# watsonyanghx/GAN_Lib_Tensorflow

Hardware: AMD Instinct MI355X
Metric: images/sec (G+D step) SNGAN-ResNet CIFAR-10 bs=64 (higher is better)
Workload: dtype bf16; 1 GPU; SNGAN ResNet CIFAR-10 32x32 bs=64 hinge: 1 G update (2x64 fakes) + 5 D updates (64 real + 64 fake) per step; global_batch=64, per_gpu_batch=64, parallelism=dp1, graphs=True, finite=True, collectives_in_graphs=False, grad_wire=fp32

## Files before the change

### gan_lib_tensorflow_amd/_lib.py

```python
import ctypes as C
import os

_HERE = os.path.dirname(os.path.abspath(__file__))
DTYPE = os.environ.get("GANK_DTYPE", "bf16").lower()
if DTYPE not in ("bf16", "fp16"):
    raise RuntimeError(f"GANK_DTYPE={DTYPE!r}: bf16 or fp16")
ACT_DTYPE_NAME = "bfloat16" if DTYPE == "bf16" else "float16"
LIB_PATH = os.path.join(_HERE, os.environ.get("GANK_LIB_NAME", "libgank.so" if DTYPE == "bf16" else "libgank_f16.so"))

P, I, L, F = C.c_void_p, C.c_int, C.c_long, C.c_float

IN_UPSAMPLE2X, IN_RELU, OUT_TANH, DY_UPSAMPLE2X, RES_UPSAMPLE2X, STATS_PREZEROED, OUT_POOLSUM2X = 1, 2, 4, 8, 64, 256, 512
STAT_SLOTS = 16


class SnDesc(C.Structure):
    _fields_ = [(n, P) for n in ("W", "u_in", "u_out", "v", "W_bar", "scal", "a", "b", "bpart",
                                 "dW_bar", "dW", "rowdot", "ga", "u_snap")] + \
               [("K", I), ("C", I), ("row_offset", I), ("chunk_offset", I)]


class WgradItem(C.Structure):
    _fields_ = [("x", P), ("dy", P), ("dw", P), ("dbias", P)]

# ... 64 lines not shown
    "gank_res8_chain_bwd_head": [C.POINTER(Res8Head), P, P, P, P, P, P, P, I, I, I, P],
    "gank_res8_conv3x3": [P, P, P, P, P, I, I, I, I, P, I, P],
    "gank_im2col_narrow": [P, P, I, I, I, I, I, I, I, I, I, I, P],
    "gank_tap_gather_up2": [P, P, P, I, I, I, I, I, I, I, I, P],
    "gank_tap_scatter_up2": [P, P, I, I, I, I, I, I, I, P],
    "gank_depth_to_space2": [P, P, I, I, I, I, P],
    "gank_space_to_depth2": [P, P, I, I, I, I, P],
    "gank_cpool_res_fprop": [P, P, P, P, P, I, I, I, I, I, I, P],
    "gank_cpool_res_dgrad": [P, P, P, P, I, I, I, I, I, P],
    "gank_cpool_res_dgrad_image_wgrad": [P, P, P, P, P, P, P, P, P, I, I, I, I, I, P, P],
    "gank_sum_slabs": [C.POINTER(SlabJob), I, P],
    "gank_convpool3x3_wgrad_job": [P, P, P, P, P, L, I, I, I, I, I, I, C.POINTER(SlabJob), P],
    "gank_conv2d_wgrad_slab_elems": [I, I, I, I, I, I, I],
    "gank_conv2d_wgrad_slabs": [P, P, P, P, I, I, I, I, I, I, I, F, P, L, C.POINTER(SlabJob), P],
    "gank_conv2d_wgrad_slab_splits": [I, I, I, I, I, I, I],
    "gank_conv2d_wgrad_slabs_rows": [P, P, P, P, I, I, I, I, I, I, I, I, F, P, L, C.POINTER(SlabJob), P],
    "gank_conv2d_wgrad_slabs_rows_tap_sums": [P, P, P, P, I, I, I, I, I, I, I, I, F, P, L, C.POINTER(SlabJob), P, I, P, P],
    "gank_conv2d_wgrad_batched_ws_elems": [I, I, I, I, I, I, I, I],
    "gank_conv2d_wgrad_batched_slabs": [C.POINTER(WgradItem), I, I, I, I, I, I, I, I, F, P, L, C.POINTER(SlabJob), P],
    "gank_deconv2d_prep_phases": [P, P, I, I, I, P],
    "gank_deconv2d_fprop": [P, P, P, P, I, I, I, I, I, I, P],
    "gank_deconv2d_dgrad": [P, P, P, I, I, I, I, I, I, P],
    "gank_deconv2d_wgrad": [P, P, P, I, I, I, I, I, I, P],
    "gank_colsum_bf16": [P, P, L, I, F, P],
    "gank_sn_ws_floats": [I, I],
    "gank_sn_power_iter_fwd": [C.POINTER(SnDesc), I, P],
    "gank_sn_power_iter_bwd": [C.POINTER(SnDesc), I, P],
    "gank_sn_power_iter_fwd_prep": [C.POINTER(SnDesc), I, C.POINTER(PrepDesc), C.POINTER(C.c_int), I, C.POINTER(LabelDenseDesc), P],
    "gank_sn_power_iter_fwd_a": [C.POINTER(SnDesc), I, P],
    "gank_sn_power_iter_fwd_b_prep": [C.POINTER(SnDesc), I, C.POINTER(PrepDesc), C.POINTER(C.c_int), I, C.POINTER(LabelDenseDesc), P, P, P, I, P],
    "gank_sn_power_iter_fwd_b_prep_feed": [C.POINTER(SnDesc), I, C.POINTER(PrepDesc), C.POINTER(C.c_int), I, C.POINTER(LabelDenseDesc), P, P, P, I,
                                           C.POINTER(CriticFeedDesc), P],
    "gank_sn_power_iter_bwd_gw": [C.POINTER(SnDesc), I, P],
    "gank_sn_adam_fwd_a": [C.POINTER(SnDesc), I, C.POINTER(C.c_void_p), P, P, P, P, L, P, P, P, P, I, P, P, P],
    "gank_label_dense_table": [P, P, P, P, P, I, I, I, P],
    "gank_concat_label_fwd": [P, P, P, P, I, I, I, I, I, P],
    "gank_concat_label_bwd": [P, P, P, I, I, I, I, P],
    "gank_label_dense_bwd": [P, P, P, P, P, P, P, I, I, I, I, P],
    "gank_label_conv3x3_bwd_pooled": [P, P, P, I, P, I, I, I, I, I, P, P, P, P, I, I, I, P],
    "gank_label_dense_bwd_parts": [P, I, P, P, P, P, P, I, I, I, P],
    "gank_sum_slabs_label_bwd": [P, I, P, P, P, I, P, I, I, I, I, I, P, P, P, I, I, I, P],
    "gank_concat_label_pool_fwd": [P, P, P, P, P, I, I, I, I, I, I, P],
    "gank_concat_label_unpool_bwd": [P, P, P, P, I, I, I, I, I, P],
    "gank_concat_label_unpool_bwd_factored": [P, P, P, P, P, I, P, P, I, I, I, I, I, I, P],
    "gank_label_conv3x3_table": [P, I, I, I, I, P, I, P, P, P, I, P, P],
    "gank_label_conv3x3_table_pooled": [P, I, I, I, I, P, I, P, P, P, I, P, P, P, I, I, I, P],
    "gank_label_conv3x3_table_pooled_shortcut": [P, I, I, I, I, P, I, P, P, P, I, P, P, P, I, I, I, P, I, P, I, P, P],
    "gank_img16_conv3x3_label_bias": [P, P, P, P, I, P, I, I, I, I, P],
    "gank_img16_conv3x3_dgrad_unpool": [P, P, P, P, I, F, P, I, I, I, P],
    "gank_img16_conv3x3_label_bwd": [P, P, P, P, I, I, I, I, P, P, I, P, I, I, I, I, P, P, P],
    "gank_label_conv3x3_bwd_ws_floats": [I, I],
    "gank_label_conv3x3_bwd": [P, P, P, I, P, I, I, I, I, I, I, I, P, P, P, P, P],
    "gank_cbn_parts": [L],
    "gank_cbn_fwd": [P, P, P, P, P, P, P, I, I, I, I, I, I, P],
    "gank_cbn_fwd_from_sums": [P, P, P, P, P, P, P, P, I, I, I, I, I, I, F, P],
    "gank_cbn_fwd_eps": [P, P, P, P, P, P, P, I, I, I, I, I, I, F, P],
    "gank_layer_norm_fwd": [P, P, P, P, P, I, I, I, F, P],
    "gank_layer_norm_bwd": [P, P, P, P, P, P, P, I, I, I, P],
    "gank_pixel_norm_fwd": [P, P, L, I, F, P],
    "gank_pixel_norm_bwd": [P, P, P, L, I, F, P],
    "gank_cbn_bwd": [P, P, P, P, P, P, P, P, P, P, I, I, I, I, I, I, P],
    "gank_cbn_stats": [P, P, P, I, I, I, I, F, P],
    "gank_cbn_stats_from_sums": [P, P, P, I, I, L, F, P],
    "gank_cbn_relu_conv3x3_fprop": [P, P, P, P, P, P, P, P, I, I, I, I, I, I, I, I, P],
    "gank_cbn_bwd_remask": [P, P, P, P, P, P, P, P, P, P, I, I, I, I, I, I, P],
    "gank_cbn_bwd_ws_floats": [I, I, I, I],
# ... 107 lines not shown
```

### gan_lib_tensorflow_amd/csrc/elementwise.hip

```cpp
#include "gank_common.h"
#include "label_conv_dev.h"

static inline dim3 grid1d(long n, int block = 256, int cap = 4096) {
  long g = (n + block - 1) / block;
  if (g > cap) g = cap;
  if (g < 1) g = 1;
  return dim3((unsigned)g);
}

#include "prep_weights.h"

__global__ void prep_wf_kernel(const float* __restrict__ w, bf16* __restrict__ wf, int K, int Cout, int CoutPad, int Kpad) {
  __shared__ float t[32][33];
  const int k0 = blockIdx.x * 32, c0 = blockIdx.y * 32;
  const int tx = threadIdx.x & 31, ty = threadIdx.x >> 5;
  for (int i = ty; i < 32; i += 8) {
    const int k = k0 + i, c = c0 + tx;
    t[i][tx] = (k < K && c < Cout) ? w[(long)k * Cout + c] : 0.f;
  }
  __syncthreads();
  for (int i = ty; i < 32; i += 8) {
    const int c = c0 + i, k = k0 + tx;
    if (c < CoutPad && k < Kpad) wf[(long)c * Kpad + k] = f2bf(t[tx][i]);
  }
}

__global__ void prep_wd_kernel(const float* __restrict__ w, bf16* __restrict__ wd, int taps, int Cin, int Cout, int CinPad, int Kpad2) {
  const long total = (long)CinPad * Kpad2;
  for (long i = blockIdx.x * (long)blockDim.x + threadIdx.x; i < total; i += (long)gridDim.x * blockDim.x) {
    const int ci = (int)(i / Kpad2), k = (int)(i - (long)ci * Kpad2);
    float v = 0.f;
    if (ci < Cin && k < taps * Cout) {
      const int tp = k / Cout, co = k - tp * Cout;
      v = w[((long)(taps - 1 - tp) * Cin + ci) * Cout + co];
// ... 820 lines not shown
    if (g < cg1) {
      bf16x8 o;
#pragma unroll
      for (int e = 0; e < 8; e++) o[e] = f2bf(v[e]);
      *reinterpret_cast<bf16x8*>(da + ((long)n * HW + r) * C1 + g * 8) = o;
    } else {
#pragma unroll
      for (int e = 0; e < 8; e++) acc[e] += bf2f(f2bf(v[e]));
    }
  }
#pragma unroll
  for (int e = 0; e < 8; e++) red[threadIdx.x * 8 + e] = acc[e];
  __syncthreads();
  for (int c = threadIdx.x; c < C2; c += NT) {
    const int gg = cg1 + (c >> 3);
    float t = 0.f;
    for (int l = 0; l < RL; l++) t += red[(l * cg + gg) * 8 + (c & 7)];
    if (de_parts > 0) {
      int lb = labels[n];
      lb = lb < 0 ? 0 : (lb >= V ? V - 1 : lb);
      if (lists[(long)lb * (N + 1) + 1] == n)
        for (int p = 0; p < de_parts; p++) t += de_add[((long)p * V + lb) * C2 + c];
    }
    de[(long)n * C2 + c] = t;
  }
  (void)cg2;
}

__global__ __launch_bounds__(1024) void label_dense_bwd_kernel(const float* __restrict__ de, const int* __restrict__ labels,
                                                               const float* __restrict__ table, const float* __restrict__ W,
                                                               float* __restrict__ dW, float* __restrict__ dbias, float* __restrict__ dtable,
                                                               int N, int V, int D, int C2, const float* __restrict__ de_add, int de_parts) {
  extern __shared__ __attribute__((aligned(16))) float lds_f[];
  float* dTg = lds_f;
  float* dT = dTg + 1024 * V;
  int* lbs = reinterpret_cast<int*>(dT + ((V * C2 + 3) & ~3));
  float* Ws = reinterpret_cast<float*>(lbs + ((N + 3) & ~3));
  float* Es = Ws + 8 * C2;
  float* dto = Es + 8 * V;
  const int tid = threadIdx.x, lane = tid & 63, wave = tid >> 6;
  const int NG = 1024 / C2, j = tid % C2, g = tid / C2;
  const int k0 = blockIdx.x * 8;
  float dw_old = 0.f, dt_old = 0.f, db_old = 0.f;
  if (dW && tid < 8 * C2 && k0 + tid / C2 < D) dw_old = dW[(long)(k0 + tid / C2) * C2 + tid % C2];
  if (dtable && tid < 8 * V && k0 + (tid & 7) < D) dt_old = dtable[(long)(tid >> 3) * D + k0 + (tid & 7)];
  if (dbias && blockIdx.x == 0 && tid < C2) db_old = dbias[tid];
  if (N == 0) {
    for (int idx = tid; idx < V * C2; idx += 1024) {
      float t = 0.f;
      for (int p = 0; p < de_parts; p++) t += de_add[(long)p * V * C2 + idx];
      dT[idx] = t;
    }
  }
  if (N > 0)
    for (int l = 0; l < V; l++) dTg[(g * V + l) * C2 + j] = 0.f;
  for (int i = tid; i < N; i += 1024) lbs[i] = labels[i];
  if (W)
    for (int i = tid; i < 8 * C2; i += 1024) { const int k = k0 + i / C2; Ws[i] = k < D ? W[(long)k * C2 + i % C2] : 0.f; }
  if (table)
    for (int i = tid; i < 8 * V; i += 1024) { const int k = k0 + (i & 7), l = i >> 3; Es[i] = k < D ? bf2f(f2bf(table[(long)l * D + k])) : 0.f; }
  __syncthreads();
  for (int nb = g; nb < N; nb += 16 * NG) {
    float x[16];
#pragma unroll
    for (int u = 0; u < 16; u++) {
      const int n = nb + u * NG;
      x[u] = n < N ? de[(long)n * C2 + j] : 0.f;
    }
#pragma unroll
    for (int u = 0; u < 16; u++) {
      const int n = nb + u * NG;
      const int l = n < N ? lbs[n] : -1;
      if (l >= 0 && l < V) dTg[(g * V + l) * C2 + j] += x[u];
    }
  }
  __syncthreads();
  if (N > 0) {
    for (int idx = tid; idx < V * C2; idx += 1024) {
      const int l = idx / C2, jj = idx % C2;
      float t = 0.f;
      for (int gg = 0; gg < NG; gg++) t += dTg[(gg * V + l) * C2 + jj];
      for (int p = 0; p < de_parts; p++) t += de_add[((long)p * V + l) * C2 + jj];
      dT[idx] = t;
    }
    __syncthreads();
  }
  if (dW)
    for (int i = tid; i < 8 * C2; i += 1024) {
      const int kk = i / C2, jj = i % C2;
      if (k0 + kk < D) {
        float t = 0.f;
        for (int l = 0; l < V; l++) t += Es[l * 8 + kk] * dT[l * C2 + jj];
        dW[(long)(k0 + kk) * C2 + jj] = (i == tid ? dw_old : dW[(long)(k0 + kk) * C2 + jj]) + t;
      }
    }
  if (dtable) {
    for (int p = wave; p < 8 * V; p += 16) {
      const int kk = p & 7, l = p >> 3;
      float t = 0.f;
      for (int jj = lane; jj < C2; jj += 64) t += dT[l * C2 + jj] * Ws[kk * C2 + jj];
      t = wave_sum(t);
      if (lane == 0) dto[p] = t;
    }
    __syncthreads();
    for (int p = tid; p < 8 * V; p += 1024) {
      const int kk = p & 7, l = p >> 3;
      if (k0 + kk < D) dtable[(long)l * D + k0 + kk] = (p == tid ? dt_old : dtable[(long)l * D + k0 + kk]) + dto[p];
    }
  }
  if (dbias && blockIdx.x == 0)
    for (int jj = tid; jj < C2; jj += 1024) {
      float t = 0.f;
      for (int l = 0; l < V; l++) t += dT[l * C2 + jj];
      dbias[jj] = (jj == tid ? db_old : dbias[jj]) + t;
    }
}

extern "C" int gank_concat_label_fwd(const void* a, const void* T, const int32_t* labels, void* y, int N, int HW, int C1, int C2, int V,
                                     void* stream) {
  GANK_REQUIRE(a && T && labels && y && N > 0 && HW > 0 && V > 0, "concat_label_fwd: bad arguments");
  GANK_REQUIRE(C1 % 8 == 0 && C2 % 8 == 0, "concat_label_fwd: channel counts must be multiples of 8");
  const long total8 = (long)N * HW * ((C1 + C2) / 8);
  hipLaunchKernelGGL(concat_label_fwd_kernel, grid1d(total8), dim3(256), 0, (hipStream_t)stream, (const bf16*)a, (const bf16*)T, labels, (bf16*)y,
                     total8, HW, C1, C2, V);
  GANK_LAUNCH_OK("concat_label_fwd");
  return 0;
}
extern "C" int gank_concat_label_bwd(const void* dy, void* da, float* de32, int N, int HW, int C1, int C2, void* stream) {
  GANK_REQUIRE(dy && da && de32 && N > 0 && HW > 0, "concat_label_bwd: bad arguments");
  GANK_REQUIRE(C1 % 8 == 0 && C2 % 8 == 0 && 1024 % (C2 / 8) == 0, "concat_label_bwd: unsupported channel counts %d,%d", C1, C2);
  hipLaunchKernelGGL(concat_label_bwd_kernel, dim3(N), dim3(1024), 0, (hipStream_t)stream, (const bf16*)dy, (bf16*)da, de32, HW, C1, C2);
  GANK_LAUNCH_OK("concat_label_bwd");
  return 0;
}
extern "C" int gank_concat_label_pool_fwd(const void* a, const void* T, const int32_t* labels, void* y, void* y_pooled, int N, int H, int W,
                                          int C1, int C2, int V, void* stream) {
  GANK_REQUIRE(a && T && labels && y_pooled && N > 0 && H > 0 && W > 0 && V > 0, "concat_label_pool_fwd: bad arguments");
  GANK_REQUIRE(C1 % 8 == 0 && C2 % 8 == 0 && H % 2 == 0 && W % 2 == 0, "concat_label_pool_fwd: channel counts must be multiples of 8, the size even");
  const long total8 = (long)N * (H / 2) * (W / 2) * ((C1 + C2) / 8);
  hipLaunchKernelGGL(concat_label_pool_fwd_kernel, grid1d(total8), dim3(256), 0, (hipStream_t)stream, (const bf16*)a, (const bf16*)T, labels,
                     (bf16*)y, (bf16*)y_pooled, total8, H / 2, W / 2, C1, C2, V);
  GANK_LAUNCH_OK("concat_label_pool_fwd");
  return 0;
}
extern "C" int gank_concat_label_unpool_bwd(const void* g_main, const void* g_pooled, void* da, float* de32, int N, int H, int W, int C1, int C2,
                                            void* stream) {
  GANK_REQUIRE(g_pooled && da && de32 && N > 0 && H > 0 && W > 0, "concat_label_unpool_bwd: bad arguments");
  GANK_REQUIRE(C1 % 8 == 0 && C2 % 8 == 0 && H % 2 == 0 && W % 2 == 0 && 1024 % ((C1 + C2) / 8) == 0,
// ... 71 lines not shown
```

### gan_lib_tensorflow_amd/csrc/sn.hip

```cpp
#include "gank_common.h"
#include "prep_weights.h"
#include "feed.h"

#define SN_MAX 16
#define SN_EPS 1e-12f
#ifndef SN_ROWS
#define SN_ROWS 32
#endif
#ifndef SN_FINE
#define SN_FINE 16
#endif

struct SnTable {
  gank_sn_desc d[SN_MAX];
  int count;
};

#define SN_TICKET_GROUPS 32
__device__ unsigned sn_tickets[SN_TICKET_GROUPS * SN_MAX];
static std::atomic<unsigned> sn_ticket_group{0};

__device__ __forceinline__ int sn_find_chunk(const SnTable& t, int chunk, int& local) {
  int w = 0;
#pragma unroll
  for (int i = 1; i < SN_MAX; i++) w += (i < t.count && chunk >= t.d[i].chunk_offset) ? 1 : 0;
  local = chunk - t.d[w].chunk_offset;
  return w;
}

__device__ __forceinline__ int sn_find_fine(const SnTable& t, int piece, int& local) {
  int w = 0;
#pragma unroll
  for (int i = 1; i < SN_MAX; i++) w += (i < t.count && piece >= t.d[i].row_offset) ? 1 : 0;
  local = piece - t.d[w].row_offset;
  return w;
// ... 846 lines not shown
                                             int prep_count, const gank_label_dense_desc* label, float* u_flat, float* u_snap_flat,
                                             const float* u_next_flat, int u_total, void* stream) {
  GANK_REQUIRE(count <= SN_MAX, "sn fwd b: at most %d weights per call", SN_MAX);
  GANK_REQUIRE(u_total == 0 || (u_flat && u_next_flat), "sn fwd b: adopting u' needs the flat u and staging buffers");
  SnAdopt ad{};
  ad.u = u_flat; ad.u_snap = u_snap_flat; ad.u_next = u_next_flat; ad.total = u_total;
  return sn_forward(table, count, prep, prep_weight, prep_count, label, (hipStream_t)stream, 2, &ad);
}

extern "C" int gank_sn_power_iter_fwd_b_prep_feed(const gank_sn_desc* table, int count, const gank_prep_desc* prep, const int* prep_weight,
                                                  int prep_count, const gank_label_dense_desc* label, float* u_flat, float* u_snap_flat,
                                                  const float* u_next_flat, int u_total, const gank_critic_feed_desc* feed, void* stream) {
  GANK_REQUIRE(count <= SN_MAX, "sn fwd b: at most %d weights per call", SN_MAX);
  GANK_REQUIRE(u_total == 0 || (u_flat && u_next_flat), "sn fwd b: adopting u' needs the flat u and staging buffers");
  GANK_REQUIRE(feed && feed->real_all && feed->labels_all && feed->fake_all && feed->both && feed->labels2 && feed->slot && feed->rng_state &&
               feed->done_counter && feed->B > 0 && feed->n_slots > 0, "sn fwd b: bad feed descriptor");
  SnAdopt ad{};
  ad.u = u_flat; ad.u_snap = u_snap_flat; ad.u_next = u_next_flat; ad.total = u_total;
  const CriticFeedArgs fd{feed->real_all, feed->labels_all, (const bf16*)feed->fake_all, (bf16*)feed->both, feed->labels2, feed->slot,
                          (unsigned long long*)feed->rng_state, feed->done_counter, feed->B, feed->n_slots, critic_feed_blocks(feed->B)};
  return sn_forward(table, count, prep, prep_weight, prep_count, label, (hipStream_t)stream, 2, &ad, &fd);
}

extern "C" int gank_sn_power_iter_bwd_gw(const gank_sn_desc* table, int count, void* stream) {
  GANK_REQUIRE(table && count > 0 && count <= SN_MAX, "sn bwd gw: 1..%d weights", SN_MAX);
  SnTable t;
  int chunks, fine;
  if (sn_fill(t, table, count, chunks, fine, true)) return 1;
  hipLaunchKernelGGL(sn_bwd_gw_kernel, dim3(fine), dim3(256), 0, (hipStream_t)stream, t);
  GANK_LAUNCH_OK("sn_power_iter_bwd_gw");
  return 0;
}

extern "C" int gank_sn_adam_fwd_a(const gank_sn_desc* table, int count, float* const* u_next, float* p, float* g, float* m, float* v, long n,
                                  float* hp, int64_t* t_state, const int64_t* iteration, uint64_t* health, int flags, int64_t* bump,
                                  const int32_t* bump_when_zero, void* stream) {
  GANK_REQUIRE(table && count > 0 && count <= SN_MAX && u_next && p && g && m && v && hp && t_state && n > 0, "sn_adam_fwd_a: bad arguments");
  SnTable t;
  int chunks, fine;
  if (sn_fill(t, table, count, chunks, fine, true)) return 1;
  SnAdamArgs ad{};
  ad.p = p; ad.g = g; ad.m = m; ad.v = v; ad.hp = hp; ad.t_state = (long long*)t_state; ad.iteration = (const long long*)iteration;
  ad.health = (unsigned long long*)health;
  ad.sn_blocks = chunks;
  ad.dw_zero = (flags & 1) ? 1 : 0;
  GANK_REQUIRE(!bump || bump_when_zero, "sn_adam_fwd_a: a counter to advance needs its condition word");
  ad.bump = (long long*)bump; ad.bump_when = bump_when_zero;
  { static const int dbg_ = gank_tune("GANK_SNTAIL_DBG", 0); ad.dbg = dbg_; }
  int order[SN_MAX];
  for (int i = 0; i < count; i++) order[i] = i;
  for (int i = 1; i < count; i++)
    for (int j = i; j > 0 && t.d[order[j]].W < t.d[order[j - 1]].W; j--) { const int x = order[j]; order[j] = order[j - 1]; order[j - 1] = x; }
  long pos = 0;
  int blocks = 0;
  for (int i = 0; i <= count; i++) {
    long lo = n, len = 0;
    if (i < count) {
      const gank_sn_desc& d = t.d[order[i]];
      GANK_REQUIRE(u_next[order[i]] && d.C <= 256, "sn_adam_fwd_a: weight %d: no staging buffer, or more than 256 columns", order[i]);
      lo = d.W - p; len = (long)d.K * d.C;
      GANK_REQUIRE(lo >= pos && lo + len <= n, "sn_adam_fwd_a: weight %d is not a disjoint view of the flat parameter buffer", order[i]);
      GANK_REQUIRE(d.dW == g + lo, "sn_adam_fwd_a: weight %d: its gradient is not the view of the flat gradient buffer at the weight's offset", order[i]);
      ad.u_next[order[i]] = u_next[order[i]];
    }
    if (lo > pos) {
      ad.gap_lo[ad.ngaps] = pos; ad.gap_hi[ad.ngaps] = lo; ad.gap_block[ad.ngaps] = blocks;
// ... 28 lines not shown
```

### gan_lib_tensorflow_amd/functional.py

```python
import torch
from torch.autograd import Function

from . import kernels as K

BF16 = K.BF16
POOL_CONV4 = True
CPOOL_RESIDENT = True
PHASE_UPCONV = True
RES8_CONV = True
UPCONV_WGRAD_PHASE = True
IMG16_CONV = True


_boundary_log = None


def boundary(x, tag):
    if _boundary_log is not None and x.requires_grad:
        _boundary_log.append((tag, x))
    return x


class record_boundaries:
    def __enter__(self):
        global _boundary_log
        self._prev, _boundary_log = _boundary_log, []
        return _boundary_log

    def __exit__(self, *exc):
        global _boundary_log
        _boundary_log = self._prev
        return False


BATCH_SMALL_WGRADS = False
_deferred = {}


def _defer_wgrad(x, g, tgt, btgt, hw, k, flags):
    _deferred.setdefault((tuple(x.shape), tuple(g.shape), hw, k, flags), []).append((x, g, tgt, btgt))


_deferred_narrow = []


def _defer_narrow(x, g, tgt, btgt, hw, k):
    _deferred_narrow.append((x, g, tgt, btgt, hw, k))


def narrow_wgrad_ok(cin, cout, k, flags_free):
    return BATCH_SMALL_WGRADS and flags_free and cin == 3 and k in (1, 3) and cout % 128 == 0


SLAB_WGRADS = True
_slab_jobs = []
LABEL_BWD_IN_SUM_SLABS = True
_label_jobs = []


def flush_wgrads():
    for (_, _, hw, k, flags), items in _deferred.items():
        K.conv2d_wgrad_batched(items, hw, k, flags, 1.0, slab_jobs=_slab_jobs if SLAB_WGRADS else None)
    _deferred.clear()
    if _slab_jobs:
        if _label_jobs and sum(c for _, c, _ in _slab_jobs) <= K.SUM_SLABS_MAX_JOBS:
            label, finish = _label_jobs.pop(0)
            finish(K.sum_slabs(_slab_jobs, label))
        else:
            K.sum_slabs(_slab_jobs)
    for label, finish in _label_jobs:
        finish(K.label_conv3x3_bwd_pooled(*label))
    _label_jobs.clear()
    while len(_deferred_narrow) >= 2:
        a, b = _deferred_narrow.pop(0), _deferred_narrow.pop(0)
        K.conv2d_wgrad_narrow_pair(a, b)
    for x, g, tgt, btgt, hw, k in _deferred_narrow:
        K.conv2d_wgrad(x, g, tgt, hw, k, 0, 1.0, dbias=btgt)
    _deferred_narrow.clear()


def reset_deferred():
    _deferred.clear()
    _deferred_narrow.clear()
    _slab_jobs.clear()
    _label_jobs.clear()


def join_wgrad():
    if _deferred or _deferred_narrow or _slab_jobs or _label_jobs:
        flush_wgrads()


def _target(p):
    mg = getattr(p, "main_grad", None)
    if mg is not None:
        return mg, True
    gb = getattr(p, "_grad_buf", None)
    if gb is not None:
        return gb, False
    return (K.zeros_f32(p.shape, p.device) if p.dtype == torch.float32 and p.is_cuda else torch.zeros_like(p)), False


def _prepared(W, k, cin, cout, want_f, want_d):
    prep = getattr(W, "_prep", None)
    if prep is not None and (not want_f or prep[0] is not None) and (not want_d or prep[1] is not None):
        return prep
    return K.prep_weights(W.detach().view(k, k, cin, cout), want_f, want_d)


def _c(t):
    return t if t.is_contiguous() else t.contiguous()


CONV1X1_BWD_ONE_LAUNCH = True
FUSE_IMAGE_WGRAD = True


class ImageWgradSink:
# ... 530 lines not shown
        g = _c(dy)
        dW = db = None
        wt = bt = None
        if ctx.needs_input_grad[1]:
            wt, acc = _target(W)
            dW = None if acc else wt
        if bias is not None and ctx.needs_input_grad[2]:
            bt, bacc = _target(bias)
            db = None if bacc else bt
        dx = K.linear_bwd(g, x, W.detach(), ctx.needs_input_grad[0], wt, bt)
        return dx, dW, db


SMALL_LINEAR_MACS = 1 << 24


def linear(x, W, bias=None):
    n = x.shape[0]
    if n * W.shape[0] * W.shape[1] <= SMALL_LINEAR_MACS:
        return _LinearSmall.apply(_c(x), W, bias)
    return _Conv2d.apply(x.view(n, 1, 1, x.shape[1]), W, bias, None, False, False, False, False).view(n, W.shape[1])


class _SpectralNorm(Function):

    @staticmethod
    def forward(ctx, batch, *Ws):
        ctx.batch = batch
        outs = batch.forward()
        return tuple(outs)

    @staticmethod
    def backward(ctx, *gs):
        join_wgrad()
        batch = ctx.batch
        tgts, rets, gl = [], [], []
        for W, g, wb in zip(batch.weights, gs, batch.W_bar):
            tgt, acc = _target(W)
            tgts.append(tgt)
            rets.append(None if acc else tgt)
            gl.append(_c(g) if g is not None else torch.zeros_like(wb))
        opt = SN_DEFER_APPLY
        if (opt is not None and batch.state is not None and batch.inplace and batch.n <= 16 and all(r is None for r in rets)
                and all(w.shape[-1] <= 256 for w in batch.weights)):
            batch.backward_gw(gl, tgts)
            opt.pending_sn = batch
        else:
            batch.backward(gl, tgts)
        return (None, *rets)


SN_DEFER_APPLY = None


class defer_sn_apply:

    def __init__(self, opt):
        self.opt = opt

    def __enter__(self):
        global SN_DEFER_APPLY
        self.prev, SN_DEFER_APPLY = SN_DEFER_APPLY, self.opt
        if self.opt is not None:
            self.opt.pending_sn = None
        return self

    def __exit__(self, *exc):
        global SN_DEFER_APPLY
        SN_DEFER_APPLY = self.prev
        return False


def spectral_norm_batch(Ws, us, snapshot=False, inplace=False, prep=None, label=None, state=None):
    batch = K.SnBatch(list(Ws), [u.detach() for u in us], snapshot, inplace, state=state)
    batch.prep, batch.label = prep, label
    outs = _SpectralNorm.apply(batch, *Ws)
    for o, wb in zip(outs, batch.W_bar):
        for attr in ("_prep", "_prep_up", "_prep_pool", "_prep_res", "_prep_cpres", "_label_T"):
            val = getattr(wb, attr, None)
            if val is not None and o is not wb:
# ... 332 lines not shown
        return K.concat_label_fwd(a, T, labels)

    @staticmethod
    def backward(ctx, dy):
        labels, table, W = ctx.saved_tensors
        bias = ctx.bias
        da, de32 = K.concat_label_bwd(_c(dy), ctx.c1)
        dt, dw, db = _label_dense_grads(ctx, de32, labels, table, W, bias)
        return (da if ctx.needs_input_grad[0] else None), None, dt, dw, db


def concat_label(a, labels, table, W, bias=None):
    return _ConcatLabel.apply(a, labels, table, W, bias)


def _label_dense_grads(ctx, de32, labels, table, W, bias, defer=False):
    need_t, need_w = ctx.needs_input_grad[2], ctx.needs_input_grad[3]
    need_b = bias is not None and ctx.needs_input_grad[4]
    dt = dw = db = None
    tt = wt = bt = None
    if need_t:
        tt, acc = _target(table)
        dt = None if acc else tt
    if need_w:
        wt, acc = _target(W)
        dw = None if acc else wt
    if need_b:
        bt, acc = _target(bias)
        db = None if acc else bt

    def finish(rows):
        if need_t or need_w or need_b:
            if labels is None:
                K.label_dense_bwd_parts(rows, table.detach(), W.detach(), wt, bt, tt)
            else:
                K.label_dense_bwd(rows, labels, table.detach(), W.detach(), wt, bt, tt)
    if defer:
        return dt, dw, db, finish
    finish(de32)
    return dt, dw, db


class _ConcatLabelForkPool(Function):

    @staticmethod
    def forward(ctx, a, labels, table, W, bias):
        ctx.set_materialize_grads(False)
        T = getattr(W, "_label_T", None)
        if T is None:
            T = K.label_dense_table(table.detach(), W.detach(), bias.detach() if bias is not None else None)
        ctx.save_for_backward(labels, table, W)
        ctx.bias = bias
        ctx.c1 = a.shape[3]
        return K.concat_label_pool_fwd(a, T, labels)

    @staticmethod
    def backward(ctx, gy, gp):
        labels, table, W = ctx.saved_tensors
        if gp is None:
            da, de32 = K.concat_label_bwd(_c(gy), ctx.c1)
        else:
            da, de32 = K.concat_label_unpool_bwd(None if gy is None else _c(gy), _c(gp), ctx.c1)
        dt, dw, db = _label_dense_grads(ctx, de32, labels, table, W, ctx.bias)
        return (da if ctx.needs_input_grad[0] else None), None, dt, dw, db


POOLED_LABEL_PART = True
# ... 457 lines not shown
```

### gan_lib_tensorflow_amd/kernels.py

```python
import ctypes as C

import torch

from . import _lib
from ._lib import IN_UPSAMPLE2X, IN_RELU, OUT_TANH, DY_UPSAMPLE2X, RES_UPSAMPLE2X, STATS_PREZEROED, OUT_POOLSUM2X, SnDesc, PrepDesc, WgradItem, LabelDenseDesc, Res8Head, SlabJob

BF16, F32, I32 = getattr(torch, _lib.ACT_DTYPE_NAME), torch.float32, torch.int32


def _stream():
    return C.c_void_p(torch.cuda.current_stream().cuda_stream)


def _p(t, dtype=None, name="tensor"):
    if t is None:
        return None
    if not t.is_cuda:
        raise RuntimeError(f"gank: {name} must live on the GPU (no CPU path exists)")
    if not t.is_contiguous():
        raise RuntimeError(f"gank: {name} must be contiguous, got strides {t.stride()} for {tuple(t.shape)}")
    if dtype is not None and t.dtype != dtype:
        raise RuntimeError(f"gank: {name} must be {dtype}, got {t.dtype}")
    return C.c_void_p(t.data_ptr())

# ... 873 lines not shown
                _lib.check(lib().gank_sn_power_iter_fwd_b_prep(*args, _stream()), "sn_power_iter_fwd_b_prep")
        else:
            if feed is not None:
                critic_feed(*feed)
            _lib.check(lib().gank_sn_power_iter_fwd_prep(self.table, self.n, ptable, pw, len(todo), C.byref(ldesc) if ldesc is not None else None,
                                                         _stream()), "sn_power_iter_fwd_prep")
        _prep_attach(self.W_bar, kinds, todo, outs)
        if self.label is not None:
            self.W_bar[self.label[1]]._label_T = self.label_out
        return self.W_bar

    def u_out_views(self):
        out, o = [], 0
        for _, c in self.KC:
            out.append(self.u_out[o:o + c])
            o += c
        return out

    def sigma(self, i):
        return self.scal[8 * i]

    def backward(self, dW_bars, dWs):
        for i, (g, d) in enumerate(zip(dW_bars, dWs)):
            self.table[i].dW_bar = _p(g, F32, "dW_bar").value
            self.table[i].dW = _p(d, F32, "dW").value
        _lib.check(lib().gank_sn_power_iter_bwd(self.table, self.n, _stream()), "sn_power_iter_bwd")

    def backward_gw(self, dW_bars, dWs):
        for i, (g, d) in enumerate(zip(dW_bars, dWs)):
            self.table[i].dW_bar = _p(g, F32, "dW_bar").value
            self.table[i].dW = _p(d, F32, "dW").value
        _lib.check(lib().gank_sn_power_iter_bwd_gw(self.table, self.n, _stream()), "sn_power_iter_bwd_gw")

    def adam_fwd_a(self, p, g, m, v, hp, t_state, iteration=None, health=None, dw_zero=False, bump=None, bump_when_zero=None):
        st = self.state
        assert st is not None and self.inplace and self.n <= 16
        ptrs = (C.c_void_p * self.n)()
        o = 0
        for i, (_, c) in enumerate(self.KC):
            ptrs[i] = st.u_next.data_ptr() + 4 * o
            o += c
        _lib.check(lib().gank_sn_adam_fwd_a(self.table, self.n, ptrs, _p(p, F32, "p"), _p(g, F32, "g"), _p(m, F32, "m"), _p(v, F32, "v"), p.numel(),
                                            _p(hp, F32, "hp"), _p(t_state, torch.int64, "t_state"), _p(iteration, torch.int64, "iteration"),
                                            _p(health, torch.int64, "health"), 1 if dw_zero else 0, _p(bump, torch.int64, "bump"),
                                            _p(bump_when_zero, I32, "bump_when_zero"), _stream()), "sn_adam_fwd_a")
        st.valid = True


def cbn_fwd(x, labels, gamma, beta, groups=1, relu=False, eps=1e-5):
    n, c = x.shape[0], x.shape[-1]
    hw = x.numel() // (n * c)
    parts = lib().gank_cbn_parts((n // groups) * hw)
    y = torch.empty_like(x)
    stats = torch.empty((groups, 2, c), dtype=F32, device=x.device)
    ws = torch.empty(groups * parts * 3 * c, dtype=F32, device=x.device)
    _lib.check(lib().gank_cbn_fwd_eps(_p(x, BF16, "x"), _p(labels, I32, "labels"), _p(gamma, F32, "gamma"), _p(beta, F32, "beta"),
                                      _p(y), _p(stats), _p(ws), n, hw, c, groups, gamma.shape[0], int(relu), float(eps), _stream()),
               "cbn_fwd")
    return y, stats


def cbn_fwd_from_sums(x, labels, gamma, beta, cs, relu=False, eps=1e-5):
    n, c = x.shape[0], x.shape[-1]
    hw = x.numel() // (n * c)
    y = torch.empty_like(x)
    stats = torch.empty((cs.groups, 2, c), dtype=F32, device=x.device)
# ... 838 lines not shown
```

### include/gank.h

```cpp
#ifndef GANK_H
#define GANK_H

#include <stddef.h>
#include <stdint.h>

#ifdef __cplusplus
extern "C" {
#endif

#define GANK_VERSION 100

#define GANK_IN_UPSAMPLE2X 1
#define GANK_IN_RELU 2
#define GANK_OUT_TANH 4
#define GANK_DY_UPSAMPLE2X 8
#define GANK_STAT_SLOTS 16
#define GANK_STATS_PREZEROED 256
#define GANK_RES_UPSAMPLE2X 64
#define GANK_OUT_POOLSUM2X 512

int gank_version(void);
int gank_act_dtype(void);
const char* gank_last_error(void);

// ... 168 lines not shown
  int chunk_offset;
} gank_sn_desc;
long gank_sn_ws_floats(int K, int C);
int gank_sn_power_iter_fwd(const gank_sn_desc* table, int count, void* stream);
int gank_sn_power_iter_bwd(const gank_sn_desc* table, int count, void* stream);
typedef struct gank_label_dense_desc {
  const float* table;
  const float* bias;
  void* out;
  int V, D;
  int weight;
} gank_label_dense_desc;
int gank_sn_power_iter_fwd_prep(const gank_sn_desc* table, int count, const gank_prep_desc* prep, const int* prep_weight,
                                int prep_count, const gank_label_dense_desc* label, void* stream);
int gank_sn_power_iter_fwd_a(const gank_sn_desc* table, int count, void* stream);
int gank_sn_power_iter_fwd_b_prep(const gank_sn_desc* table, int count, const gank_prep_desc* prep, const int* prep_weight,
                                  int prep_count, const gank_label_dense_desc* label, float* u_flat, float* u_snap_flat,
                                  const float* u_next_flat, int u_total, void* stream);
typedef struct gank_critic_feed_desc {
  const uint8_t* real_all;
  const int32_t* labels_all;
  const void* fake_all;
  void* both;
  int32_t* labels2;
  int32_t* slot;
  uint64_t* rng_state;
  uint32_t* done_counter;
  int B, n_slots;
} gank_critic_feed_desc;
int gank_sn_power_iter_fwd_b_prep_feed(const gank_sn_desc* table, int count, const gank_prep_desc* prep, const int* prep_weight,
                                       int prep_count, const gank_label_dense_desc* label, float* u_flat, float* u_snap_flat,
                                       const float* u_next_flat, int u_total, const gank_critic_feed_desc* feed, void* stream);
int gank_sn_power_iter_bwd_gw(const gank_sn_desc* table, int count, void* stream);
int gank_sn_adam_fwd_a(const gank_sn_desc* table, int count, float* const* u_next, float* p, float* g, float* m, float* v, long n,
                       float* hp, int64_t* t_state, const int64_t* iteration, uint64_t* health, int flags, int64_t* bump,
                       const int32_t* bump_when_zero, void* stream);

int gank_cbn_parts(long rows_per_group);
int gank_cbn_fwd(const void* x, const int32_t* labels, const float* gamma, const float* beta, void* y,
                 float* stats, float* ws, int N, int HW, int C, int groups, int n_labels, int relu, void* stream);
int gank_cbn_fwd_eps(const void* x, const int32_t* labels, const float* gamma, const float* beta, void* y,
                     float* stats, float* ws, int N, int HW, int C, int groups, int n_labels, int relu, float eps, void* stream);
int gank_cbn_fwd_from_sums(const void* x, const int32_t* labels, const float* gamma, const float* beta, void* y, float* stats,
                           const float* sums, const float* shift, int N, int HW, int C, int groups, int n_labels, int relu,
                           float eps, void* stream);
int gank_cbn_stats(const void* x, float* stats, float* ws, int N, int HW, int C, int groups, float eps, void* stream);
int gank_cbn_stats_from_sums(const float* sums, const float* shift, float* stats, int C, int groups, long rows_per_group,
                             float eps, void* stream);
int gank_cbn_relu_conv3x3_fprop(const void* x, const int32_t* labels, const float* gamma, const float* beta, const float* stats,
                                const void* wf, const float* bias, void* y, int N, int H, int W, int Cin, int Cout,
                                int groups, int n_labels, int flags, void* stream);
int gank_cbn_bwd(const void* dy, const void* x, const void* y, const int32_t* labels, const float* gamma,
                 const float* stats, void* dx, float* dgamma, float* dbeta, float* ws, int N, int HW, int C,
                 int groups, int n_labels, int relu, void* stream);
int gank_cbn_bwd_remask(const void* dy, const void* x, const float* beta, const int32_t* labels, const float* gamma,
                        const float* stats, void* dx, float* dgamma, float* dbeta, float* ws, int N, int HW, int C,
                        int groups, int n_labels, int relu, void* stream);
long gank_cbn_bwd_ws_floats(int N, int HW, int C, int groups);
int gank_cbn_bwd_ws(const void* dy, const void* x, const void* y, const float* beta, const int32_t* labels, const float* gamma,
                    const float* stats, void* dx, float* dgamma, float* dbeta, float* ws, long ws_floats, int N, int HW, int C,
                    int groups, int n_labels, int relu, void* stream);

int gank_layer_norm_fwd(const void* x, const float* gamma, const float* beta, void* y, float* stats, int N, int HW, int C,
                        float eps, void* stream);
int gank_layer_norm_bwd(const void* dy, const void* x, const float* gamma, const float* stats, void* dx, float* dgamma,
                        float* dbeta, int N, int HW, int C, void* stream);
// ... 166 lines not shown
```

Before: 61880 images/sec.

## Fuse critic label-dense backward into spectral-norm gradient dot kernel

Defers the critic's label-dense backward (the parts-based path) and runs it inside a new combined kernel. That kernel also computes the spectral-norm W·dW_bar partial dot products for all weights, and for the dense layer it takes them straight from the freshly written dW. This removes one kernel launch and one re-read of the dense weight gradient per critic backward. In exchange it adds a ticket-based last-block reduction, Python-side holding state, and shape restrictions with fallback to the old two-launch path.

```diff
diff --git a/gan_lib_tensorflow_amd/_lib.py b/gan_lib_tensorflow_amd/_lib.py
--- a/gan_lib_tensorflow_amd/_lib.py
+++ b/gan_lib_tensorflow_amd/_lib.py
@@ -120,6 +120,7 @@
     "gank_sn_power_iter_fwd_b_prep_feed": [C.POINTER(SnDesc), I, C.POINTER(PrepDesc), C.POINTER(C.c_int), I, C.POINTER(LabelDenseDesc), P, P, P, I,
                                            C.POINTER(CriticFeedDesc), P],
     "gank_sn_power_iter_bwd_gw": [C.POINTER(SnDesc), I, P],
+    "gank_sn_bwd_gw_label_dense": [C.POINTER(SnDesc), I, I, P, I, P, P, P, P, I, P],
     "gank_sn_adam_fwd_a": [C.POINTER(SnDesc), I, C.POINTER(C.c_void_p), P, P, P, P, L, P, P, P, P, I, P, P, P],
     "gank_label_dense_table": [P, P, P, P, P, I, I, I, P],
     "gank_concat_label_fwd": [P, P, P, P, I, I, I, I, I, P],
diff --git a/gan_lib_tensorflow_amd/csrc/elementwise.hip b/gan_lib_tensorflow_amd/csrc/elementwise.hip
--- a/gan_lib_tensorflow_amd/csrc/elementwise.hip
+++ b/gan_lib_tensorflow_amd/csrc/elementwise.hip
@@ -1,5 +1,6 @@
 #include "gank_common.h"
 #include "label_conv_dev.h"
+#include "label_dense_dev.h"
 
 static inline dim3 grid1d(long n, int block = 256, int cap = 4096) {
   long g = (n + block - 1) / block;
@@ -886,88 +887,7 @@
                                                                float* __restrict__ dW, float* __restrict__ dbias, float* __restrict__ dtable,
                                                                int N, int V, int D, int C2, const float* __restrict__ de_add, int de_parts) {
   extern __shared__ __attribute__((aligned(16))) float lds_f[];
-  float* dTg = lds_f;
-  float* dT = dTg + 1024 * V;
-  int* lbs = reinterpret_cast<int*>(dT + ((V * C2 + 3) & ~3));
-  float* Ws = reinterpret_cast<float*>(lbs + ((N + 3) & ~3));
-  float* Es = Ws + 8 * C2;
-  float* dto = Es + 8 * V;
-  const int tid = threadIdx.x, lane = tid & 63, wave = tid >> 6;
-  const int NG = 1024 / C2, j = tid % C2, g = tid / C2;
-  const int k0 = blockIdx.x * 8;
-  float dw_old = 0.f, dt_old = 0.f, db_old = 0.f;
-  if (dW && tid < 8 * C2 && k0 + tid / C2 < D) dw_old = dW[(long)(k0 + tid / C2) * C2 + tid % C2];
-  if (dtable && tid < 8 * V && k0 + (tid & 7) < D) dt_old = dtable[(long)(tid >> 3) * D + k0 + (tid & 7)];
-  if (dbias && blockIdx.x == 0 && tid < C2) db_old = dbias[tid];
-  if (N == 0) {
-    for (int idx = tid; idx < V * C2; idx += 1024) {
-      float t = 0.f;
-      for (int p = 0; p < de_parts; p++) t += de_add[(long)p * V * C2 + idx];
-      dT[idx] = t;
-    }
-  }
-  if (N > 0)
-    for (int l = 0; l < V; l++) dTg[(g * V + l) * C2 + j] = 0.f;
-  for (int i = tid; i < N; i += 1024) lbs[i] = labels[i];
-  if (W)
-    for (int i = tid; i < 8 * C2; i += 1024) { const int k = k0 + i / C2; Ws[i] = k < D ? W[(long)k * C2 + i % C2] : 0.f; }
-  if (table)
-    for (int i = tid; i < 8 * V; i += 1024) { const int k = k0 + (i & 7), l = i >> 3; Es[i] = k < D ? bf2f(f2bf(table[(long)l * D + k])) : 0.f; }
-  __syncthreads();
-  for (int nb = g; nb < N; nb += 16 * NG) {
-    float x[16];
-#pragma unroll
-    for (int u = 0; u < 16; u++) {
-      const int n = nb + u * NG;
-      x[u] = n < N ? de[(long)n * C2 + j] : 0.f;
-    }
-#pragma unroll
-    for (int u = 0; u < 16; u++) {
-      const int n = nb + u * NG;
-      const int l = n < N ? lbs[n] : -1;
-      if (l >= 0 && l < V) dTg[(g * V + l) * C2 + j] += x[u];
-    }
-  }
-  __syncthreads();
-  if (N > 0) {
-    for (int idx = tid; idx < V * C2; idx += 1024) {
-      const int l = idx / C2, jj = idx % C2;
-      float t = 0.f;
-      for (int gg = 0; gg < NG; gg++) t += dTg[(gg * V + l) * C2 + jj];
-      for (int p = 0; p < de_parts; p++) t += de_add[((long)p * V + l) * C2 + jj];
-      dT[idx] = t;
-    }
-    __syncthreads();
-  }
-  if (dW)
-    for (int i = tid; i < 8 * C2; i += 1024) {
-      const int kk = i / C2, jj = i % C2;
-      if (k0 + kk < D) {
-        float t = 0.f;
-        for (int l = 0; l < V; l++) t += Es[l * 8 + kk] * dT[l * C2 + jj];
-        dW[(long)(k0 + kk) * C2 + jj] = (i == tid ? dw_old : dW[(long)(k0 + kk) * C2 + jj]) + t;
-      }
-    }
-  if (dtable) {
-    for (int p = wave; p < 8 * V; p += 16) {
-      const int kk = p & 7, l = p >> 3;
-      float t = 0.f;
-      for (int jj = lane; jj < C2; jj += 64) t += dT[l * C2 + jj] * Ws[kk * C2 + jj];
-      t = wave_sum(t);
-      if (lane == 0) dto[p] = t;
-    }
-    __syncthreads();
-    for (int p = tid; p < 8 * V; p += 1024) {
-      const int kk = p & 7, l = p >> 3;
-      if (k0 + kk < D) dtable[(long)l * D + k0 + kk] = (p == tid ? dt_old : dtable[(long)l * D + k0 + kk]) + dto[p];
-    }
-  }
-  if (dbias && blockIdx.x == 0)
-    for (int jj = tid; jj < C2; jj += 1024) {
-      float t = 0.f;
-      for (int l = 0; l < V; l++) t += dT[l * C2 + jj];
-      dbias[jj] = (jj == tid ? db_old : dbias[jj]) + t;
-    }
+  label_dense_bwd_block(de, labels, table, W, dW, dbias, dtable, N, V, D, C2, de_add, de_parts, blockIdx.x, lds_f, nullptr);
 }
 
 extern "C" int gank_concat_label_fwd(const void* a, const void* T, const int32_t* labels, void* y, int N, int HW, int C1, int C2, int V,
diff --git a/gan_lib_tensorflow_amd/csrc/label_dense_dev.h b/gan_lib_tensorflow_amd/csrc/label_dense_dev.h
--- /dev/null
+++ b/gan_lib_tensorflow_amd/csrc/label_dense_dev.h
@@ -0,0 +1,96 @@
+#pragma once
+#include "gank_common.h"
+
+__device__ __forceinline__ float label_dense_bwd_block(const float* __restrict__ de, const int* __restrict__ labels,
+                                                       const float* __restrict__ table, const float* __restrict__ W,
+                                                       float* __restrict__ dW, float* __restrict__ dbias, float* __restrict__ dtable,
+                                                       int N, int V, int D, int C2, const float* __restrict__ de_add, int de_parts,
+                                                       int block, float* lds_f, const float* __restrict__ Wm) {
+  float* dTg = lds_f;
+  float* dT = dTg + 1024 * V;
+  int* lbs = reinterpret_cast<int*>(dT + ((V * C2 + 3) & ~3));
+  float* Ws = reinterpret_cast<float*>(lbs + ((N + 3) & ~3));
+  float* Es = Ws + 8 * C2;
+  float* dto = Es + 8 * V;
+  const int tid = threadIdx.x, lane = tid & 63, wave = tid >> 6;
+  const int NG = 1024 / C2, j = tid % C2, g = tid / C2;
+  const int k0 = block * 8;
+  float dw_old = 0.f, dt_old = 0.f, db_old = 0.f;
+  if (dW && tid < 8 * C2 && k0 + tid / C2 < D) dw_old = dW[(long)(k0 + tid / C2) * C2 + tid % C2];
+  float wm_old = 0.f, prod = 0.f;
+  if (Wm && dW && tid < 8 * C2 && k0 + tid / C2 < D) wm_old = Wm[(long)(k0 + tid / C2) * C2 + tid % C2];
+  if (dtable && tid < 8 * V && k0 + (tid & 7) < D) dt_old = dtable[(long)(tid >> 3) * D + k0 + (tid & 7)];
+  if (dbias && block == 0 && tid < C2) db_old = dbias[tid];
+  if (N == 0) {
+    for (int idx = tid; idx < V * C2; idx += 1024) {
+      float t = 0.f;
+      for (int p = 0; p < de_parts; p++) t += de_add[(long)p * V * C2 + idx];
+      dT[idx] = t;
+    }
+  }
+  if (N > 0)
+    for (int l = 0; l < V; l++) dTg[(g * V + l) * C2 + j] = 0.f;
+  for (int i = tid; i < N; i += 1024) lbs[i] = labels[i];
+  if (W)
+    for (int i = tid; i < 8 * C2; i += 1024) { const int k = k0 + i / C2; Ws[i] = k < D ? W[(long)k * C2 + i % C2] : 0.f; }
+  if (table)
+    for (int i = tid; i < 8 * V; i += 1024) { const int k = k0 + (i & 7), l = i >> 3; Es[i] = k < D ? bf2f(f2bf(table[(long)l * D + k])) : 0.f; }
+  __syncthreads();
+  for (int nb = g; nb < N; nb += 16 * NG) {
+    float x[16];
+#pragma unroll
+    for (int u = 0; u < 16; u++) {
+      const int n = nb + u * NG;
+      x[u] = n < N ? de[(long)n * C2 + j] : 0.f;
+    }
+#pragma unroll
+    for (int u = 0; u < 16; u++) {
+      const int n = nb + u * NG;
+      const int l = n < N ? lbs[n] : -1;
+      if (l >= 0 && l < V) dTg[(g * V + l) * C2 + j] += x[u];
+    }
+  }
+  __syncthreads();
+  if (N > 0) {
+    for (int idx = tid; idx < V * C2; idx += 1024) {
+      const int l = idx / C2, jj = idx % C2;
+      float t = 0.f;
+      for (int gg = 0; gg < NG; gg++) t += dTg[(gg * V + l) * C2 + jj];
+      for (int p = 0; p < de_parts; p++) t += de_add[((long)p * V + l) * C2 + jj];
+      dT[idx] = t;
+    }
+    __syncthreads();
+  }
+  if (dW)
+    for (int i = tid; i < 8 * C2; i += 1024) {
+      const int kk = i / C2, jj = i % C2;
+      if (k0 + kk < D) {
+        float t = 0.f;
+        for (int l = 0; l < V; l++) t += Es[l * 8 + kk] * dT[l * C2 + jj];
+        const float nv = (i == tid ? dw_old : dW[(long)(k0 + kk) * C2 + jj]) + t;
+        dW[(long)(k0 + kk) * C2 + jj] = nv;
+        if (i == tid) prod = nv * wm_old;
+      }
+    }
+  if (dtable) {
+    for (int p = wave; p < 8 * V; p += 16) {
+      const int kk = p & 7, l = p >> 3;
+      float t = 0.f;
+      for (int jj = lane; jj < C2; jj += 64) t += dT[l * C2 + jj] * Ws[kk * C2 + jj];
+      t = wave_sum(t);
+      if (lane == 0) dto[p] = t;
+    }
+    __syncthreads();
+    for (int p = tid; p < 8 * V; p += 1024) {
+      const int kk = p & 7, l = p >> 3;
+      if (k0 + kk < D) dtable[(long)l * D + k0 + kk] = (p == tid ? dt_old : dtable[(long)l * D + k0 + kk]) + dto[p];
+    }
+  }
+  if (dbias && block == 0)
+    for (int jj = tid; jj < C2; jj += 1024) {
+      float t = 0.f;
+      for (int l = 0; l < V; l++) t += dT[l * C2 + jj];
+      dbias[jj] = (jj == tid ? db_old : dbias[jj]) + t;
+    }
+  return prod;
+}
diff --git a/gan_lib_tensorflow_amd/csrc/sn.hip b/gan_lib_tensorflow_amd/csrc/sn.hip
--- a/gan_lib_tensorflow_amd/csrc/sn.hip
+++ b/gan_lib_tensorflow_amd/csrc/sn.hip
@@ -1,6 +1,7 @@
 #include "gank_common.h"
 #include "prep_weights.h"
 #include "feed.h"
+#include "label_dense_dev.h"
 
 #define SN_MAX 16
 #define SN_EPS 1e-12f
@@ -913,6 +914,121 @@
   return 0;
 }
 
+struct SnGwDense {
+  const float* de_add;
+  const float* table;
+  const float* W;
+  float* dbias;
+  float* dtable;
+  float* part;
+  int parts, V, wi, dense_blocks, nfine_total;
+};
+__device__ float sn_dense_part[SN_TICKET_GROUPS * 64];
+
+__global__ __launch_bounds__(1024) void sn_bwd_gw_label_dense_kernel(SnTable t, SnGwDense q, unsigned* __restrict__ ticket) {
+  extern __shared__ __attribute__((aligned(16))) float lds_f[];
+  __shared__ float red[16];
+  __shared__ int flag;
+  const int tid = threadIdx.x;
+  if ((int)blockIdx.x >= q.dense_blocks) {
+    const int grp = tid >> 8, gt = tid & 255;
+    const int piece = ((int)blockIdx.x - q.dense_blocks) * 4 + grp;
+    const bool live = piece < q.nfine_total;
+    int ch;
+    const int wi = sn_find_fine(t, live ? piece : q.nfine_total - 1, ch);
+    const gank_sn_desc& d = t.d[wi];
+    const bool work = live && wi != q.wi;
+    const int K = d.K, C = d.C, k0 = ch * SN_FINE, kn = min(SN_FINE, K - k0), nch = (K + SN_ROWS - 1) / SN_ROWS;
+    const float* __restrict__ W = d.W + (long)k0 * C;
+    const float* __restrict__ G = d.dW_bar + (long)k0 * C;
+    const int total = work ? kn * C : 0;
+    float s = 0.f;
+    if ((C & 3) == 0 && sn_al16(d.W) && sn_al16(d.dW_bar)) {
+      constexpr int NB = 4;
+      f32x4 w[NB], g[NB];
+      const int n4 = total >> 2;
+      for (int base = 0; base < n4; base += NB * 256) {
+#pragma unroll
+        for (int i = 0; i < NB; i++) {
+          const int qi = base + i * 256 + gt;
+          const f32x4 z = {0.f, 0.f, 0.f, 0.f};
+          w[i] = qi < n4 ? reinterpret_cast<const f32x4*>(W)[qi] : z;
+          g[i] = qi < n4 ? reinterpret_cast<const f32x4*>(G)[qi] : z;
+        }
+#pragma unroll
+        for (int i = 0; i < NB; i++) s += ((w[i][0] * g[i][0] + w[i][1] * g[i][1]) + w[i][2] * g[i][2]) + w[i][3] * g[i][3];
+      }
+    } else {
+      for (int qi = gt; qi < total; qi += 256) s += W[qi] * G[qi];
+    }
+    s = wave_sum(s);
+    if ((tid & 63) == 0) red[tid >> 6] = s;
+    __syncthreads();
+    if (gt == 0 && work) {
+      float tt = 0.f;
+      for (int i = 0; i < 4; i++) tt += red[grp * 4 + i];
+      d.bpart[(long)nch * C + nch + ch] = tt;
+    }
+    return;
+  }
+  const gank_sn_desc& d = t.d[q.wi];
+  const int D = d.K, C2 = d.C, nch = (D + SN_ROWS - 1) / SN_ROWS, nfine = (D + SN_FINE - 1) / SN_FINE;
+  const float prod = label_dense_bwd_block(nullptr, nullptr, q.table, q.W, const_cast<float*>(d.dW_bar), q.dbias, q.dtable, 0, q.V, D, C2,
+                                           q.de_add, q.parts, blockIdx.x, lds_f, d.W);
+  const float bs = block_sum(prod, red);
+  if (tid == 0) {
+    sn_store_wt(q.part + blockIdx.x, bs);
+    asm volatile("s_waitcnt vmcnt(0)" ::: "memory");
+    const unsigned tk = __hip_atomic_fetch_add(ticket, 1u, __ATOMIC_RELAXED, __HIP_MEMORY_SCOPE_AGENT);
+    const int last = tk == (unsigned)(q.dense_blocks - 1);
+    if (last) {
+      __hip_atomic_store(ticket, 0u, __ATOMIC_RELAXED, __HIP_MEMORY_SCOPE_AGENT);
+      __builtin_amdgcn_fence(__ATOMIC_ACQUIRE, "agent");
+    }
+    flag = last;
+  }
+  __syncthreads();
+  if (!flag) return;
+  if (tid < nfine) {
+    const float p0 = __hip_atomic_load(q.part + 2 * tid, __ATOMIC_RELAXED, __HIP_MEMORY_SCOPE_AGENT);
+    const float p1 = 2 * tid + 1 < q.dense_blocks ? __hip_atomic_load(q.part + 2 * tid + 1, __ATOMIC_RELAXED, __HIP_MEMORY_SCOPE_AGENT) : 0.f;
+    d.bpart[(long)nch * C2 + nch + tid] = p0 + p1;
+  }
+}
+
+extern "C" int gank_sn_bwd_gw_label_dense(const gank_sn_desc* table, int count, int dense_weight, const float* de_parts_rows, int parts,
+                                          const float* emb_table, const float* W_bar, float* dbias, float* dtable, int V, void* stream) {
+  static_assert(SN_FINE == 16, "two 8-row blocks of the dense layer's backward per fine piece");
+  GANK_REQUIRE(table && count > 0 && count <= SN_MAX && dense_weight >= 0 && dense_weight < count, "sn_bwd_gw_label_dense: 1..%d weights, one of them the dense layer", SN_MAX);
+  GANK_REQUIRE(de_parts_rows && parts > 0 && emb_table && V > 0 && (!dtable || W_bar), "sn_bwd_gw_label_dense: bad arguments");
+  SnTable t;
+  int chunks, fine;
+  if (sn_fill(t, table, count, chunks, fine, true)) return 1;
+  const gank_sn_desc& d = t.d[dense_weight];
+  const int D = d.K, C2 = d.C, dense_blocks = cdiv(D, 8);
+  GANK_REQUIRE(8 * C2 <= 1024 && 1024 % C2 == 0 && dense_blocks <= 64, "sn_bwd_gw_label_dense: a dense layer of %d x %d is not supported (C2 <= 128 dividing 1024, D <= 512)", D, C2);
+  const size_t lds = (1024 * (size_t)V + (((size_t)V * C2 + 3) & ~(size_t)3) + 8 * (size_t)C2 + 16 * (size_t)V) * 4;
+  GANK_REQUIRE(lds <= 156 * 1024, "sn_bwd_gw_label_dense: V = %d labels do not fit the LDS", V);
+  GANK_MAX_DYNAMIC_LDS(sn_bwd_gw_label_dense_kernel, 156 * 1024, "sn_bwd_gw_label_dense");
+  unsigned* tickets_base = sn_ticket_base();
+  if (!tickets_base) return gank_set_error("sn_bwd_gw_label_dense: ticket words not found");
+  static std::atomic<float*> part_addr[64];
+  int dev = 0;
+  (void)hipGetDevice(&dev);
+  float* part_base = part_addr[dev & 63].load(std::memory_order_relaxed);
+  if (!part_base) {
+    if (hipGetSymbolAddress(reinterpret_cast<void**>(&part_base), HIP_SYMBOL(sn_dense_part)) != hipSuccess || !part_base)
+      return gank_set_error("sn_bwd_gw_label_dense: workspace not found");
+    part_addr[dev & 63].store(part_base, std::memory_order_relaxed);
+  }
+  const unsigned group = sn_ticket_group.fetch_add(1, std::memory_order_relaxed) % SN_TICKET_GROUPS;
+  const SnGwDense q{de_parts_rows, emb_table, W_bar, dbias, dtable, part_base + group * 64, parts, V, dense_weight, dense_blocks, fine};
+  hipLaunchKernelGGL(sn_bwd_gw_label_dense_kernel, dim3(dense_blocks + (fine + 3) / 4), dim3(1024), lds, (hipStream_t)stream, t, q,
+                     tickets_base + group * SN_MAX);
+  GANK_LAUNCH_OK("sn_bwd_gw_label_dense");
+  return 0;
+}
+
 extern "C" int gank_sn_adam_fwd_a(const gank_sn_desc* table, int count, float* const* u_next, float* p, float* g, float* m, float* v, long n,
                                   float* hp, int64_t* t_state, const int64_t* iteration, uint64_t* health, int flags, int64_t* bump,
                                   const int32_t* bump_when_zero, void* stream) {
diff --git a/gan_lib_tensorflow_amd/functional.py b/gan_lib_tensorflow_amd/functional.py
--- a/gan_lib_tensorflow_amd/functional.py
+++ b/gan_lib_tensorflow_amd/functional.py
@@ -56,6 +56,9 @@
 _slab_jobs = []
 LABEL_BWD_IN_SUM_SLABS = True
 _label_jobs = []
+FUSE_CRITIC_TAIL = True
+_hold_dense = [False]
+_held_dense = []
 
 
 def flush_wgrads():
@@ -84,6 +87,8 @@
     _deferred_narrow.clear()
     _slab_jobs.clear()
     _label_jobs.clear()
+    _held_dense.clear()
+    _hold_dense[0] = False
 
 
 def join_wgrad():
@@ -680,8 +685,13 @@
 
     @staticmethod
     def backward(ctx, *gs):
-        join_wgrad()
         batch = ctx.batch
+        _hold_dense[0] = FUSE_CRITIC_TAIL and SN_DEFER_APPLY is not None and batch.n <= 16
+        try:
+            join_wgrad()
+        finally:
+            _hold_dense[0] = False
+        held = _held_dense.pop() if _held_dense else None
         tgts, rets, gl = [], [], []
         for W, g, wb in zip(batch.weights, gs, batch.W_bar):
             tgt, acc = _target(W)
@@ -691,9 +701,17 @@
         opt = SN_DEFER_APPLY
         if (opt is not None and batch.state is not None and batch.inplace and batch.n <= 16 and all(r is None for r in rets)
                 and all(w.shape[-1] <= 256 for w in batch.weights)):
-            batch.backward_gw(gl, tgts)
+            if held is not None and batch.backward_gw_label_dense(gl, tgts, *held):
+                held = None
+            else:
+                if held is not None:
+                    K.label_dense_bwd_parts(*held)
+                    held = None
+                batch.backward_gw(gl, tgts)
             opt.pending_sn = batch
         else:
+            if held is not None:
+                K.label_dense_bwd_parts(*held)
             batch.backward(gl, tgts)
         return (None, *rets)
 
@@ -1092,7 +1110,10 @@
     def finish(rows):
         if need_t or need_w or need_b:
             if labels is None:
-                K.label_dense_bwd_parts(rows, table.detach(), W.detach(), wt, bt, tt)
+                if _hold_dense[0] and not _held_dense:
+                    _held_dense.append((rows, table.detach(), W.detach(), wt, bt, tt))
+                else:
+                    K.label_dense_bwd_parts(rows, table.detach(), W.detach(), wt, bt, tt)
             else:
                 K.label_dense_bwd(rows, labels, table.detach(), W.detach(), wt, bt, tt)
     if defer:
diff --git a/gan_lib_tensorflow_amd/kernels.py b/gan_lib_tensorflow_amd/kernels.py
--- a/gan_lib_tensorflow_amd/kernels.py
+++ b/gan_lib_tensorflow_amd/kernels.py
@@ -929,6 +929,23 @@
             self.table[i].dW = _p(d, F32, "dW").value
         _lib.check(lib().gank_sn_power_iter_bwd_gw(self.table, self.n, _stream()), "sn_power_iter_bwd_gw")
 
+    def backward_gw_label_dense(self, dW_bars, dWs, parts, table, w_bar, dw, dbias, dtable):
+        idx = [i for i, g in enumerate(dW_bars) if dw is not None and g.data_ptr() == dw.data_ptr()]
+        if len(idx) != 1 or table is None:
+            return False
+        d, c2 = self.KC[idx[0]]
+        if tuple(dw.shape) != (d, c2) or tuple(w_bar.shape) != (d, c2) or c2 > 128 or 1024 % c2 or d > 512 or parts.shape[2] != c2:
+            return False
+        for i, (g, t) in enumerate(zip(dW_bars, dWs)):
+            self.table[i].dW_bar = _p(g, F32, "dW_bar").value
+            self.table[i].dW = _p(t, F32, "dW").value
+        npart, v, _ = parts.shape
+        assert tuple(table.shape) == (v, d)
+        _lib.check(lib().gank_sn_bwd_gw_label_dense(self.table, self.n, idx[0], _p(parts, F32, "parts"), npart, _p(table, F32, "table"),
+                                                    _p(w_bar, F32, "w_bar"), _p(dbias, F32, "dbias"), _p(dtable, F32, "dtable"), v, _stream()),
+                   "sn_bwd_gw_label_dense")
+        return True
+
     def adam_fwd_a(self, p, g, m, v, hp, t_state, iteration=None, health=None, dw_zero=False, bump=None, bump_when_zero=None):
         st = self.state
         assert st is not None and self.inplace and self.n <= 16
diff --git a/include/gank.h b/include/gank.h
--- a/include/gank.h
+++ b/include/gank.h
@@ -224,6 +224,8 @@
                                        int prep_count, const gank_label_dense_desc* label, float* u_flat, float* u_snap_flat,
                                        const float* u_next_flat, int u_total, const gank_critic_feed_desc* feed, void* stream);
 int gank_sn_power_iter_bwd_gw(const gank_sn_desc* table, int count, void* stream);
+int gank_sn_bwd_gw_label_dense(const gank_sn_desc* table, int count, int dense_weight, const float* de_parts_rows, int parts,
+                               const float* emb_table, const float* W_bar, float* dbias, float* dtable, int V, void* stream);
 int gank_sn_adam_fwd_a(const gank_sn_desc* table, int count, float* const* u_next, float* p, float* g, float* m, float* v, long n,
                        float* hp, int64_t* t_state, const int64_t* iteration, uint64_t* health, int flags, int64_t* bump,
                        const int32_t* bump_when_zero, void* stream);
```

New measurement: 62080 images/sec (median of 6 runs). Within noise of the previous version (+0.3%).
